# HKUDS/LLMRec

Measured on AMD Instinct MI355X. Metric: bpr_train_edges_per_sec, higher is better.
Workload: dtype f32

## Files before the change

include/llmrec_hip.h:

```cpp
#ifndef LLMREC_HIP_H
#define LLMREC_HIP_H

#include <stdint.h>

#ifdef __cplusplus
extern "C" {
#endif

#define LLMREC_ABI_VERSION 8

enum {
    LLMREC_OK = 0,
    LLMREC_EINVAL = -1,
    LLMREC_EHIP = -2,
    LLMREC_EWORKSPACE = -3,
    LLMREC_EUNSUPPORTED = -4
};

typedef void* llmrec_stream_t;

int llmrec_abi_version(void);
const char* llmrec_status_string(int status);
const char* llmrec_last_error(void);

// ... 27 lines not shown
    int32_t op; float alpha;
    const float* Z; int64_t ldz;
    const float* S; int64_t lds;
    const float* post_scale;
    const uint8_t* x_row_mask; int32_t x_mask_active; uint8_t* y_row_flag; const uint8_t* z_row_flag; const uint8_t* y_row_gate;
    const uint8_t* y_row_needed; int32_t rows_listed_only;
    const int32_t* x_mask_stamp; int32_t mask_from_slice;
} llmrec_spmm_epilogue_t;
#define LLMREC_SORT_UNIQUE_MAX 32768
#define LLMREC_SPMM_COMPACT_PARTS 8
int llmrec_sort_unique_ids_i32(int64_t n, const int64_t* ids, int32_t* list, int32_t* n_out, llmrec_stream_t stream);
int64_t llmrec_spmm_rows_compact_workspace_bytes(int64_t capacity, int32_t d);
int llmrec_spmm_rows_compact_f32(int64_t n_rows, int64_t n_cols, const int32_t* rowptr, const int32_t* colidx, const float* row_scale,
                                 const float* X, int64_t ldx, int32_t d, const int32_t* row_list, const int32_t* n_list_dev, int32_t capacity,
                                 float* out, int64_t ldo, void* workspace, int64_t workspace_bytes, llmrec_stream_t stream);
int llmrec_scatter_set_rows_f32(int32_t capacity, const int32_t* row_list, const int32_t* n_list_dev, int32_t d, const float* src, int64_t lds,
                                float* dst, int64_t ldd, llmrec_stream_t stream);
int llmrec_mark_rows_u8(int64_t n, const int64_t* ids, int32_t value, uint8_t* flags, llmrec_stream_t stream);
int llmrec_mark_neighbours_u8(int64_t n, const int64_t* ids, const int32_t* rowptr, const int32_t* colidx, int32_t value, uint8_t* flags,
                              llmrec_stream_t stream);
int llmrec_batch_reach_rows(int64_t n_users, int64_t n_items, const int64_t* users, const int64_t* pos, const int64_t* neg, int32_t B_cap,
                            const int32_t* n_valid, const int32_t* item_rowptr, const int32_t* item_colidx, uint8_t* flags,
                            int32_t* row_list, int32_t* n_rows, llmrec_stream_t stream);

int llmrec_spmm_plan_count(int64_t n_rows, const int32_t* rowptr, int32_t t_wave, int32_t t_block, int32_t segment,
                           int32_t* scratch4 , int32_t* counts_host, llmrec_stream_t stream);
int llmrec_spmm_plan_fill(int64_t n_rows, const int32_t* rowptr, int32_t t_wave, int32_t t_block, int32_t segment,
                          int32_t* scratch4, int32_t* wave_rows, int32_t* block_rows, int32_t* split_rows,
                          int32_t* split_seg_begin, int32_t* seg_split, llmrec_stream_t stream);

int llmrec_csr_permute_rows(int64_t n_rows, const int32_t* rowptr, const int32_t* colidx, const int32_t* perm, const int32_t* p_rowptr,
                            int32_t* p_colidx, llmrec_stream_t stream);

int llmrec_spmm_f32(int64_t n_rows, int64_t n_cols,
                    const int32_t* rowptr, const int32_t* colidx, const float* val,
                    const float* row_scale, const float* col_scale,
                    const float* X, int64_t ldx, float* Y, int64_t ldy, int32_t d, int32_t slice_width,
                    const llmrec_spmm_plan_t* plan_host, float* partials,
                    const llmrec_spmm_epilogue_t* epilogue_host , llmrec_stream_t stream);

int llmrec_rows_to_bf16(int64_t n_rows, int32_t d, const float* row_scale ,
                        const float* X, int64_t ldx, uint16_t* Xb, int64_t ldxb, llmrec_stream_t stream);
int llmrec_spmm_xbf16_f32(int64_t n_rows, int64_t n_cols, const int32_t* rowptr, const int32_t* colidx, const float* val,
                          const float* row_scale, const float* col_scale,
                          const uint16_t* Xb, int64_t ldxb,
                          float* Y, int64_t ldy,
// ... 437 lines not shown
```

llmrec_amd/csrc/guests.h:

```cpp
#pragma once
#include "common.h"
#include "reach.h"

namespace llmrec {

__device__ __forceinline__ int bpr_batch(const int32_t* n_valid_dev, int B_max) {
    int B = n_valid_dev ? n_valid_dev[0] : B_max;
    return B > B_max ? B_max : (B < 0 ? 0 : B);
}

struct Philox {
    uint32_t key[2];
    __device__ Philox(uint64_t seed) { key[0] = (uint32_t)seed; key[1] = (uint32_t)(seed >> 32); }
    __device__ void operator()(uint32_t c0, uint32_t c1, uint32_t c2, uint32_t c3, uint32_t out[4]) const {
        uint32_t k0 = key[0], k1 = key[1];
#pragma unroll
        for (int r = 0; r < 10; ++r) {
            const uint64_t p0 = (uint64_t)0xD2511F53u * c0, p1 = (uint64_t)0xCD9E8D57u * c2;
            const uint32_t n0 = (uint32_t)(p1 >> 32) ^ c1 ^ k0, n1 = (uint32_t)p1;
            const uint32_t n2 = (uint32_t)(p0 >> 32) ^ c3 ^ k1, n3 = (uint32_t)p0;
            c0 = n0; c1 = n1; c2 = n2; c3 = n3;
            k0 += 0x9E3779B9u; k1 += 0xBB67AE85u;
        }
        out[0] = c0; out[1] = c1; out[2] = c2; out[3] = c3;
// ... 186 lines not shown
        below += kj < me; lower_id += idj < id; same_id += idj == id;
    }
    below = (int)group_sum<16>((float)below); lower_id = (int)group_sum<16>((float)lower_id); same_id = (int)group_sum<16>((float)same_id);
    if (gl == 0) {
        const int base = items ? B_max : 0;
        plan[base + below] = me;
        int32_t* runlen = reinterpret_cast<int32_t*>(plan + 3 * (int64_t)B_max);
        runlen[base + below] = (below == lower_id && id != PLAN_NO_ID) ? same_id : 0;
    }
}

struct PlanReachArgs {
    const int64_t* users;
    const int64_t* pos;
    const int64_t* neg;
    int B_max;
    const int32_t* n_valid_dev;
    uint64_t* plan;
    int plan_blocks;
    int64_t n_users, n_items;
    const int32_t* item_rowptr;
    const int32_t* item_colidx;
    uint8_t* flags;
};

template <int NT>
__device__ __forceinline__ void guest_block(const PlanReachArgs& a, int vb, char* smem) {
    if (vb < a.plan_blocks)
        bpr_plan_block<NT>(vb, reinterpret_cast<uint64_t*>(smem), a.users, a.pos, a.neg, a.B_max, a.n_valid_dev, a.plan);
    else
        batch_reach_mark_block<NT>(vb - a.plan_blocks, a.B_max, a.n_valid_dev, a.users, a.pos, a.neg, a.n_users, a.n_items, a.item_rowptr,
                                   a.item_colidx, a.flags);
}

static inline int guest_prepare(const llmrec_guest_plan_reach_t& g, int nt, const char* who, PlanReachArgs& a, int64_t& blocks, size_t& shmem) {
    blocks = 0; shmem = 0;
    LLMREC_CHECK_ARG(g.B_max >= 0 && g.n_users > 0 && g.n_users < 0x7fffffffll && g.n_items > 0, "%s: bad sizes", who);
    LLMREC_CHECK_ARG(g.item_rowptr && g.item_colidx && g.flags, "%s: null pointer", who);
    if (g.B_max > LLMREC_BPR_MAX_B) { set_error("%s: B_max %d > %d", who, g.B_max, LLMREC_BPR_MAX_B); return LLMREC_EUNSUPPORTED; }
    if (g.B_max == 0) return LLMREC_OK;
    LLMREC_CHECK_ARG(g.users && g.pos && g.neg && g.plan, "%s: null pointer", who);
    const int plan_blocks = (int)plan_blocks_for(g.B_max, nt);
    blocks = plan_blocks + reach_mark_blocks(g.B_max, nt);
    shmem = sizeof(uint64_t) * 2 * (size_t)g.B_max;
    a = PlanReachArgs{g.users, g.pos, g.neg, g.B_max, g.n_valid_dev, g.plan, plan_blocks, g.n_users, g.n_items, g.item_rowptr, g.item_colidx,
                      g.flags};
    return LLMREC_OK;
}

struct LossW { float w[LLMREC_BPR_MAX_PROBLEMS]; };
constexpr int LA_SLOTS = 1024;
constexpr int LA_TREES = 4 * LLMREC_BPR_MAX_PROBLEMS + 1;
__device__ __forceinline__ float wave_tree_sum_1024(const float* __restrict__ src, int n, int lane) {
    float r[16];
#pragma unroll
    for (int j = 0; j < 16; ++j) r[j] = 0.f;
    for (int base = 0; base < n; base += LA_SLOTS) {
        float x[16];
#pragma unroll
        for (int j = 0; j < 16; ++j) { const int b = base + lane + 64 * j; x[j] = b < n ? src[b] : 0.f; }
#pragma unroll
        for (int j = 0; j < 16; ++j) { const int b = base + lane + 64 * j; if (b < n) r[j] += x[j]; }
    }
#pragma unroll
    for (int h = 8; h > 0; h >>= 1) {
#pragma unroll
        for (int j = 0; j < h; ++j) r[j] += r[j + h];
    }
    float x = r[0];
// ... 89 lines not shown
```

llmrec_amd/csrc/reach.h:

```cpp
#pragma once
#include "common.h"

namespace llmrec {

constexpr int REACH_SPLIT = 8;

static inline int64_t reach_mark_blocks(int B_cap, int nt = 256) { return ceil_div(3 * (int64_t)B_cap * REACH_SPLIT, nt / 64); }

template <int NT = 256>
__device__ __forceinline__ void batch_reach_mark_block(int vb, int B_cap, const int32_t* __restrict__ n_valid, const int64_t* __restrict__ users,
                                                       const int64_t* __restrict__ pos, const int64_t* __restrict__ neg, int64_t n_users,
                                                       int64_t n_items, const int32_t* __restrict__ rowptr, const int32_t* __restrict__ colidx,
                                                       uint8_t* __restrict__ flags) {
    const int w = vb * (NT / 64) + (threadIdx.x >> 6), lane = threadIdx.x & 63;
    int nv = n_valid ? *n_valid : B_cap;
    nv = nv < B_cap ? nv : B_cap;
    const int part = w % REACH_SPLIT, job = w / REACH_SPLIT;
    const int b = job / 3, role = job - 3 * b;
    if (b >= nv) return;
    if (role == 0) {
        const int64_t u = users[b];
        if (part == 0 && lane == 0 && u >= 0 && u < n_users) flags[u] = 1;
        return;
    }
    const int64_t it = role == 1 ? pos[b] : neg[b];
    if (it < 0 || it >= n_items) return;
    const int32_t s = rowptr[it], e = rowptr[it + 1];
    for (int32_t k = s + part * 64 + lane; k < e; k += 64 * REACH_SPLIT) flags[colidx[k]] = 1;
}

}
```

llmrec_amd/csrc/rowops.hip:

```cpp
#include "common.h"
#include "adamw.h"
#include "reach.h"
#include <type_traits>

namespace llmrec {

constexpr int RL = 16;
constexpr int ROWS_PER_BLOCK = 256 / RL;

template <int VEC, int NCHUNK>
struct RowReg {
    float x[NCHUNK][VEC];
    __device__ __forceinline__ void load(const float* row, int gl, int d) {
#pragma unroll
        for (int k = 0; k < NCHUNK; ++k) {
            const int c = (k * RL + gl) * VEC;
            if (VEC == 4) {
                float4 v = (c < d) ? *reinterpret_cast<const float4*>(row + c) : make_float4(0.f, 0.f, 0.f, 0.f);
                x[k][0] = v.x; x[k][1 % VEC] = v.y; x[k][2 % VEC] = v.z; x[k][3 % VEC] = v.w;
            } else {
                x[k][0] = (c < d) ? row[c] : 0.f;
            }
        }
    }
    __device__ __forceinline__ void store(float* row, int gl, int d) const {
#pragma unroll
// ... 580 lines not shown
    for (int c = gl; c < d; c += 16) dot = fmaf(y[c], alpha * g[c], dot);
    dot = group_sum<16>(dot);
    const float ps = post_scale ? post_scale[row] : 1.0f;
    float* o = dZ + row * lddz;
    for (int c = gl; c < d; c += 16) o[c] = ps * (y[c] * (alpha * g[c] - dot));
}

constexpr int MARK_SPLIT = 32;
__global__ __launch_bounds__(256) void mark_neighbours_kernel(int64_t n, const int64_t* __restrict__ ids, const int32_t* __restrict__ rowptr,
                                                              const int32_t* __restrict__ colidx, uint8_t value, uint8_t* __restrict__ flags) {
    const int64_t w = (int64_t)blockIdx.x * 4 + (threadIdx.x >> 6);
    const int64_t j = w / MARK_SPLIT;
    const int part = (int)(w - j * MARK_SPLIT);
    if (j >= n) return;
    const int64_t row = ids[j];
    if (row < 0) return;
    const int32_t s = rowptr[row], e = rowptr[row + 1];
    for (int64_t k = (int64_t)s + part * 64 + (threadIdx.x & 63); k < e; k += 64 * MARK_SPLIT) flags[colidx[k]] = value;
}

__global__ __launch_bounds__(256) void batch_reach_mark_kernel(int B_cap, const int32_t* __restrict__ n_valid, const int64_t* __restrict__ users,
                                                               const int64_t* __restrict__ pos, const int64_t* __restrict__ neg, int64_t n_users,
                                                               int64_t n_items, const int32_t* __restrict__ rowptr, const int32_t* __restrict__ colidx,
                                                               uint8_t* __restrict__ flags) {
    batch_reach_mark_block((int)blockIdx.x, B_cap, n_valid, users, pos, neg, n_users, n_items, rowptr, colidx, flags);
}

__global__ __launch_bounds__(1024) void flags_compact_kernel(int64_t n, uint8_t* __restrict__ flags, int32_t* __restrict__ list, int32_t* __restrict__ n_out) {
    __shared__ int32_t wave_total[16];
    const int tid = threadIdx.x, lane = tid & 63, wave = tid >> 6;
    const int64_t per = ((n + 1023) / 1024 + 15) / 16 * 16;
    const int64_t r0 = tid * per, r1 = r0 + per < n ? r0 + per : n;
    int32_t c = 0;
    for (int64_t r = r0; r < r1; r += 16) {
        const uint4 v = *reinterpret_cast<const uint4*>(flags + r);
        const uint32_t wd[4] = {v.x, v.y, v.z, v.w};
#pragma unroll
        for (int q = 0; q < 4; ++q)
#pragma unroll
            for (int bb = 0; bb < 4; ++bb)
                c += (r + 4 * q + bb < r1) && ((wd[q] >> (8 * bb)) & 0xffu);
    }
    int32_t incl = c;
#pragma unroll
    for (int off = 1; off < 64; off <<= 1) {
        const int32_t v = __shfl_up(incl, off, 64);
        if (lane >= off) incl += v;
    }
    if (lane == 63) wave_total[wave] = incl;
    __syncthreads();
    int32_t base = 0, total = 0;
#pragma unroll
// ... 60 lines not shown
            for (int j = 0; j < COMPACT_WPT; ++j) {
                const uint32_t wd[4] = {v[j].x, v[j].y, v[j].z, v[j].w};
                if ((wd[0] | wd[1] | wd[2] | wd[3]) == 0u) continue;
                const int64_t r = 16 * (mine + j);
#pragma unroll
                for (int q = 0; q < 4; ++q)
#pragma unroll
                    for (int bb = 0; bb < 4; ++bb)
                        if ((wd[q] >> (8 * bb)) & 0xffu) list[o++] = (int32_t)(r + 4 * q + bb);
                const int64_t left = n - r;
                if (left >= 16) *reinterpret_cast<uint4*>(flags + r) = uint4{0u, 0u, 0u, 0u};
                else for (int64_t bb = 0; bb < left; ++bb) flags[r + bb] = 0;
            }
        }
        done += total;
    }
    const int32_t pad_end = (done + 15) / 16 * 16 + 16;
    for (int32_t k = done + tid; k < pad_end; k += 256) list[k] = 0;
    if (tid == 0) *n_out = done;
}

template <int VEC, int NCHUNK>
__global__ __launch_bounds__(256) void fuse_fwd_multi_compact_kernel(int d, FuseMulti m, int64_t n_flags, uint8_t* __restrict__ flags,
                                                                     int32_t* __restrict__ list, int32_t* __restrict__ n_out) {
    __shared__ float ss_red[256];
    if (blockIdx.x == 0) { flags_compact_block256(n_flags, flags, list, n_out, reinterpret_cast<int32_t*>(ss_red)); return; }
    fuse_fwd_multi_block<VEC, NCHUNK>((int)blockIdx.x - 1, (int)gridDim.x - 1, d, m, ss_red);
}

constexpr int COLSUM_BLOCKS = 128;
constexpr int COLSUM_MAX_D = 64 * LLMREC_COLSUM_MAX_GROUPS;
__global__ __launch_bounds__(256) void colsum_partial_kernel(int64_t rows, int d, const float* __restrict__ X, int64_t ldx,
                                                             const float* __restrict__ w, float* __restrict__ partial) {
    float acc[COLSUM_MAX_D / 256] = {};
    for (int64_t r = blockIdx.x; r < rows; r += gridDim.x) {
        const float wr = w ? w[r] : 1.f;
        const float* row = X + r * ldx;
#pragma unroll
        for (int k = 0; k < COLSUM_MAX_D / 256; ++k) {
            const int c = k * 256 + threadIdx.x;
            if (c < d) acc[k] = fmaf(wr, row[c], acc[k]);
        }
    }
#pragma unroll
    for (int k = 0; k < COLSUM_MAX_D / 256; ++k) {
        const int c = k * 256 + threadIdx.x;
        if (c < d) partial[(int64_t)blockIdx.x * d + c] = acc[k];
    }
}
struct ColsumGroups { float* out[LLMREC_COLSUM_MAX_GROUPS]; int n_groups; };
// ... 13 lines not shown
    __syncthreads();
    if (c >= gw) return;
    for (int q = 0; q < g.n_groups; ++q) {
        bool first = true;
        for (int e = 0; e < q; ++e) first = first && g.out[e] != g.out[q];
        float* o = g.out[q] + c;
        *o = (first && !accumulate) ? col[gw * q + c] : *o + col[gw * q + c];
    }
}

struct GatherTerms { const float* t[LLMREC_MAX_TERMS]; int64_t ld[LLMREC_MAX_TERMS]; int n; };

__global__ __launch_bounds__(256) void gather_mean_kernel(int64_t n, const int64_t* __restrict__ idx, int d, float scale, GatherTerms g,
                                                          float* __restrict__ out, int64_t ldo) {
    const int gl = threadIdx.x & 15;
    const int64_t b = (int64_t)blockIdx.x * 16 + (threadIdx.x >> 4);
    if (b >= n) return;
    const int64_t row = idx[b];
    for (int c = gl; c < d; c += 16) {
        float s = 0.f;
        for (int t = 0; t < g.n; ++t) s += g.t[t][row * g.ld[t] + c];
        out[b * ldo + c] = scale * s;
    }
}

extern "C" {

int llmrec_softmax_rows_fwd_f32(int64_t rows, int32_t d, const float* Z, int64_t ldz, float* Y, int64_t ldy,
                                llmrec_stream_t stream_) {
    hipStream_t stream = (hipStream_t)stream_;
    LLMREC_CHECK_ARG(rows >= 0 && d > 0, "softmax_fwd: bad sizes");
    if (rows == 0) return LLMREC_OK;
    LLMREC_CHECK_ARG(Z && Y && ldz >= d && ldy >= d, "softmax_fwd: null pointer or ld < d");
    const bool vec4 = d % 4 == 0 && ldz % 4 == 0 && ldy % 4 == 0 && aligned16(Z) && aligned16(Y);
    const int grid = grid_for(rows, ROWS_PER_BLOCK);
    int rc = dispatch_rows(d, vec4,
        [&](auto nc) { softmax_fwd_kernel<4, decltype(nc)::value><<<grid, 256, 0, stream>>>(rows, d, Z, ldz, Y, ldy); return 0; },
        [&](auto nc) { softmax_fwd_kernel<1, decltype(nc)::value><<<grid, 256, 0, stream>>>(rows, d, Z, ldz, Y, ldy); return 0; });
    if (rc) return rc;
    LLMREC_LAUNCH_CHECK();
    return LLMREC_OK;
}

int llmrec_softmax_rows_bwd_scaled_f32(int64_t rows, int32_t d, float alpha, const float* Y, int64_t ldy, const float* dY, int64_t lddy,
                                       float* dZ, int64_t lddz, llmrec_stream_t stream_) {
    hipStream_t stream = (hipStream_t)stream_;
// ... 123 lines not shown
        vec4 = vec4 && q.ldo % 4 == 0 && aligned16(q.out);
        for (int i = 0; i < q.n_mean; ++i) {
            LLMREC_CHECK_ARG(q.mean_terms[i] && q.mean_ld[i] >= d, "fuse_fwd_multi: problem %d: bad mean term %d", k, i);
            a.mean_terms[i] = q.mean_terms[i]; a.mean_ld[i] = q.mean_ld[i];
            vec4 = vec4 && q.mean_ld[i] % 4 == 0 && aligned16(q.mean_terms[i]);
        }
        for (int i = 0; i < q.n_norm; ++i) {
            LLMREC_CHECK_ARG(q.norm_terms[i] && q.norm_ld[i] >= d, "fuse_fwd_multi: problem %d: bad norm term %d", k, i);
            a.norm_terms[i] = q.norm_terms[i]; a.norm_ld[i] = q.norm_ld[i]; a.rates[i] = q.rates[i];
            vec4 = vec4 && q.norm_ld[i] % 4 == 0 && aligned16(q.norm_terms[i]);
        }
        m.rows[k] = q.rows; m.out[k] = q.out; m.ldo[k] = q.ldo;
        blocks[k] = q.rows > 0 ? grid_for(q.rows, ROWS_PER_BLOCK) : 0;
    }
    m.block_begin = blocks[0];
    const int grid = blocks[0] + blocks[1];
    if (n_sumsq_terms > 0) {
        for (int k = 0; k < n_problems; ++k) LLMREC_CHECK_ARG(n_sumsq_terms <= p[k].n_norm, "fuse_fwd_multi: problem %d has fewer than %d norm terms", k, n_sumsq_terms);
        if (grid > partial_capacity) { set_error("fuse_fwd_multi: %d partial sums > capacity %d", grid, partial_capacity); return LLMREC_EWORKSPACE; }
        *n_partial_host = grid;
        m.n_sumsq = n_sumsq_terms; m.sumsq_partial = sumsq_partial;
    }
    if (flags) {
        int rc = dispatch_rows(d, vec4,
            [&](auto nc) { fuse_fwd_multi_compact_kernel<4, decltype(nc)::value><<<grid + 1, 256, 0, stream>>>(d, m, n_flags, flags, row_list, n_rows); return 0; },
            [&](auto) { set_error("fuse_fwd_multi_sumsq_compact: d = %d with rows that are not 16-byte aligned", d); return (int)LLMREC_EUNSUPPORTED; });
        if (rc) return rc;
        LLMREC_LAUNCH_CHECK();
        return LLMREC_OK;
    }
    if (grid == 0) return LLMREC_OK;
    int rc = dispatch_rows(d, vec4,
        [&](auto nc) { fuse_fwd_multi_kernel<4, decltype(nc)::value><<<grid, 256, 0, stream>>>(d, m); return 0; },
        [&](auto nc) { fuse_fwd_multi_kernel<1, decltype(nc)::value><<<grid, 256, 0, stream>>>(d, m); return 0; });
    if (rc) return rc;
    LLMREC_LAUNCH_CHECK();
    return LLMREC_OK;
}

int llmrec_fuse_fwd_multi_sumsq_f32(int32_t n_problems, const llmrec_fuse_fwd_problem_t* p, int32_t d, int32_t n_sumsq_terms,
                                    float* sumsq_partial, int32_t partial_capacity, int32_t* n_partial_host, llmrec_stream_t stream_) {
    return fuse_fwd_multi_launch(n_problems, p, d, n_sumsq_terms, sumsq_partial, partial_capacity, n_partial_host, 0, nullptr, nullptr, nullptr,
                                 (hipStream_t)stream_);
}

int llmrec_fuse_fwd_multi_sumsq_compact_f32(int32_t n_problems, const llmrec_fuse_fwd_problem_t* p, int32_t d, int32_t n_sumsq_terms,
                                            float* sumsq_partial, int32_t partial_capacity, int32_t* n_partial_host,
                                            int64_t n_users, uint8_t* flags, int32_t* row_list, int32_t* n_rows, llmrec_stream_t stream_) {
// ... 231 lines not shown
    LLMREC_CHECK_ARG(row_list && n_list_dev && src && dst && lds_ >= d && ldd >= d, "scatter_set_rows: null pointer or ld < d");
    scatter_set_rows_kernel<<<(unsigned)ceil_div(capacity, 16), 256, 0, (hipStream_t)stream_>>>(capacity, row_list, n_list_dev, d, src, lds_, dst, ldd);
    LLMREC_LAUNCH_CHECK();
    return LLMREC_OK;
}

int llmrec_mark_rows_u8(int64_t n, const int64_t* ids, int32_t value, uint8_t* flags, llmrec_stream_t stream_) {
    LLMREC_CHECK_ARG(n >= 0 && value >= 0 && value <= 255, "mark_rows: bad argument");
    if (n == 0) return LLMREC_OK;
    LLMREC_CHECK_ARG(ids && flags, "mark_rows: null pointer");
    LLMREC_CHECK_ARG(n / 256 < 0x7fffffffll, "mark_rows: too many rows for one launch");
    mark_rows_kernel<<<(unsigned)ceil_div(n, 256), 256, 0, (hipStream_t)stream_>>>(n, ids, (uint8_t)value, flags);
    LLMREC_LAUNCH_CHECK();
    return LLMREC_OK;
}

int llmrec_batch_reach_rows(int64_t n_users, int64_t n_items, const int64_t* users, const int64_t* pos, const int64_t* neg, int32_t B_cap,
                            const int32_t* n_valid, const int32_t* item_rowptr, const int32_t* item_colidx, uint8_t* flags,
                            int32_t* row_list, int32_t* n_rows, llmrec_stream_t stream_) {
    LLMREC_CHECK_ARG(n_users > 0 && n_users < 0x7fffffffll && n_items > 0 && B_cap >= 0, "batch_reach_rows: bad sizes");
    LLMREC_CHECK_ARG(users && pos && neg && item_rowptr && item_colidx && flags && row_list && n_rows, "batch_reach_rows: null pointer");
    LLMREC_CHECK_ARG((uintptr_t)flags % 16 == 0, "batch_reach_rows: flags must be 16-byte aligned (and readable up to n_users rounded up to 16 bytes)");
    hipStream_t stream = (hipStream_t)stream_;
    if (B_cap > 0) {
        batch_reach_mark_kernel<<<(unsigned)reach_mark_blocks(B_cap), 256, 0, stream>>>(B_cap, n_valid, users, pos, neg, n_users, n_items,
                                                                                                item_rowptr, item_colidx, flags);
        LLMREC_LAUNCH_CHECK();
    }
    flags_compact_kernel<<<1, 1024, 0, stream>>>(n_users, flags, row_list, n_rows);
    LLMREC_LAUNCH_CHECK();
    return LLMREC_OK;
}

int llmrec_softmax_rows_bwd_listed_f32(int64_t n, const int64_t* ids, int32_t d, float alpha, const float* Y, int64_t ldy,
                                       const float* dY, int64_t lddy, const float* post_scale, float* dZ, int64_t lddz,
                                       llmrec_stream_t stream_) {
    LLMREC_CHECK_ARG(n >= 0 && d > 0, "softmax_bwd_listed: bad sizes");
    if (n == 0) return LLMREC_OK;
    LLMREC_CHECK_ARG(ids && Y && dY && dZ && ldy >= d && lddy >= d && lddz >= d, "softmax_bwd_listed: null pointer or ld < d");
    softmax_bwd_listed_kernel<<<(unsigned)ceil_div(n, 16), 256, 0, (hipStream_t)stream_>>>(n, ids, d, alpha, Y, ldy, dY, lddy, post_scale, dZ, lddz);
    LLMREC_LAUNCH_CHECK();
    return LLMREC_OK;
}

int llmrec_mark_neighbours_u8(int64_t n, const int64_t* ids, const int32_t* rowptr, const int32_t* colidx, int32_t value, uint8_t* flags,
                              llmrec_stream_t stream_) {
    LLMREC_CHECK_ARG(n >= 0 && value >= 0 && value <= 255, "mark_neighbours: bad argument");
    if (n == 0) return LLMREC_OK;
    LLMREC_CHECK_ARG(ids && rowptr && colidx && flags, "mark_neighbours: null pointer");
    LLMREC_CHECK_ARG(n * MARK_SPLIT / 4 < 0x7fffffffll, "mark_neighbours: too many rows for one launch");
    mark_neighbours_kernel<<<(unsigned)ceil_div(n * MARK_SPLIT, 4), 256, 0, (hipStream_t)stream_>>>(n, ids, rowptr, colidx, (uint8_t)value, flags);
    LLMREC_LAUNCH_CHECK();
    return LLMREC_OK;
// ... 85 lines not shown
```

llmrec_amd/fused.py:

```python
from __future__ import annotations

import contextlib
import ctypes
import gc
from collections import namedtuple
from itertools import zip_longest
from typing import Callable, Optional

import torch

from . import _lib, ops, step_options
from .engine import Hyper

_p, _ld, _c = ops._p, ops._ld, ctypes


def _call(name, *a):
    _lib.call(name, *a, ops._stream())


def _raw(args):
    return [_p(a) if a is None or isinstance(a, torch.Tensor) else a for a in args]


@contextlib.contextmanager
def _capture_without_gc(graph, multi_branch: bool):
    from . import require_graph_replay
# ... 130 lines not shown
        if self.restore:
            if decoder is None or user_targets is None or item_targets is None or feat_loss_type not in ops.RESTORE_LOSS_TYPES:
                raise RuntimeError("FusedStep: the restoration term needs the decoder, both target sets and feat_loss_type sce or mse")
            if d != 64 or S > 2 + _lib.CONST["LLMREC_MASK_MAX_TENSORS"]:
                raise RuntimeError("FusedStep: the restoration launches are compiled for d = 64 and at most %d attribute streams"
                                   % _lib.CONST["LLMREC_MASK_MAX_TENSORS"])
            as_target = lambda x: torch.as_tensor(x).detach().to(device=dev, dtype=torch.float32).contiguous()
            self.decoder, self.feat_loss_type, self.alpha_l = decoder, feat_loss_type, float(alpha_l)
            self.user_targets, self.item_targets = as_target(user_targets), [as_target(item_targets[k]) for k in self.keys]
            self.re_rows_u, self.re_rows_i = f(self.m_users), f(len(self.keys) * self.m_items)
            self.re_vals = z(1 + len(self.keys))
        if not self.preprop:
            self.P_cat, self.dP_cat = f(I, S * d), f(I, S * d)
        else:
            item_feats = [model.image_feats, model.text_feats] + [model.item_feats[k] for k in self.keys]
            self.AX = [self._propagate_constant(self.ui.fwd, x) for x in item_feats]
            self.a_rowsum = ops.spmm_raw(self.ui.fwd, torch.ones(I, 4, dtype=torch.float32, device=dev))[:, 0].contiguous()
            self.ws_colsum = torch.empty(_lib.query("llmrec_weighted_colsum_workspace_bytes", S * d), dtype=torch.uint8, device=dev)
        if self.wgrad_rows:
            self.act_flags = torch.zeros(U + 16, dtype=torch.uint8, device=dev)[:U]
            self.act_rows = torch.zeros(U + 32, dtype=torch.int32, device=dev)
            self.act_n = torch.zeros(1, dtype=torch.int32, device=dev)
            self.act_expected = None
        if self.fold:
            self.ss_cap = 2 * 2048
            self.ss_partial = torch.zeros(self.ss_cap, dtype=torch.float32, device=dev)
            self.ss_n = 0
        self._refuse_guests = False
        self._block_slots = 2 * torch.cuda.get_device_properties(dev).multi_processor_count
        self._emb_params = [model.user_id_embedding.weight, model.item_id_embedding.weight]
        self._lin_params = [p for p in optimizer.params if p.grad is not None and all(p is not e for e in self._emb_params)]

    @staticmethod
    def _propagate_constant(a: ops.Csr, X: torch.Tensor) -> torch.Tensor:
        X = X.detach()
        out = torch.empty(a.n_rows, X.shape[1], dtype=torch.float32, device=X.device)
        step = 64 if X.shape[1] % 64 == 0 else X.shape[1]
        for c0 in range(0, X.shape[1], step):
            ops.spmm_raw(a, X[:, c0:c0 + step], out=out[:, c0:c0 + step])
        return out

    def _fork(self, *streams):
        if self.multi_stream:
            cur = torch.cuda.current_stream()
            for st in streams:
                st.wait_stream(cur)
# ... 90 lines not shown
    def _linear(self, X, lin, out):
        _call("llmrec_linear_fwd_f32", X.shape[0], self.d, X.shape[1], _p(X), _ld(X), _p(lin.weight), _ld(lin.weight), _p(lin.bias),
              _p(out), _ld(out))

    def projection_jobs(self):
        m = self.m
        if self.preprop:
            lins = [m.image_trans, m.text_trans] + [m.item_trans] * len(self.keys)
            jobs = [(self.AX[s_], lins[s_], self._side(self.U_cat, s_), self.a_rowsum) for s_ in range(self.S)]
        else:
            jobs = [(m.item_feats[key], m.item_trans, self._side(self.P_cat, 2 + k), None) for k, key in enumerate(self.keys)]
            jobs += [(m.text_feats, m.text_trans, self._side(self.P_cat, 1), None), (m.image_feats, m.image_trans, self._side(self.P_cat, 0), None)]
        jobs.append((m.user_feats, m.user_trans, self.P_usr, None))
        jobs.sort(key=lambda j: -j[0].shape[1])
        return jobs

    def wgrad_targets(self, dY_cat, dP_usr):
        m = self.m
        if self.preprop:
            feats, roww = self.AX, self.a_rowsum
        else:
            feats, roww = [m.image_feats, m.text_feats] + [m.item_feats[key] for key in self.keys], None
        rows = (self.act_rows, self.act_n, self.act_expected) if self.wgrad_rows else None
        item_pairs = [(self._side(dY_cat, 2 + k), feats[2 + k], roww, rows) for k in range(len(self.keys))]
        return [(item_pairs, m.item_trans.weight.grad, m.item_trans.bias.grad, False),
                ([(dP_usr, m.user_feats)], m.user_trans.weight.grad, m.user_trans.bias.grad, False),
                ([(self._side(dY_cat, 1), feats[1], roww)], m.text_trans.weight.grad, m.text_trans.bias.grad, False),
                ([(self._side(dY_cat, 0), feats[0], roww)], m.image_trans.weight.grad, m.image_trans.bias.grad, False)]

    def _project_all(self):
        jobs = self.projection_jobs()
        if self.d > 64 or len(jobs) > _lib.CONST["LLMREC_LINEAR_MAX_PROBLEMS"]:
            if self.preprop:
                raise RuntimeError("FusedStep: the pre-propagated projection needs the grouped launch (d <= 64); set LLMREC_PREPROPAGATE=0")
            for X, lin, out, _ in jobs:
                self._linear(X, lin, out)
            return
        arr = self._projection_problems(jobs)
        _call("llmrec_linear_fwd_grouped_bf16x3" if self.gemm == "bf16x3" else "llmrec_linear_fwd_grouped_f32", len(jobs), arr, self.d)

    @staticmethod
    def _projection_problems(jobs):
        return ops.linear_problems([(X, lin.weight, lin.bias, out, bscale) for X, lin, out, bscale in jobs])

    def _project_all_hosting(self, job) -> bool:
        a, X, Y, kw = job
        jobs = self.projection_jobs()
        if not (self.host_chain and not self._refuse_guests and not self.multi_stream and self.gemm == "bf16x3" and self.d == 64
                and len(jobs) <= _lib.CONST["LLMREC_LINEAR_MAX_PROBLEMS"] and a.nnz < ops.SPMM_LATENCY_NNZ
# ... 441 lines not shown
        if main_first:
            self._spmm_jobs(side)
            self._fork_from(ev_fuse, self.s1)
        else:
            self._fork(self.s1)
        if loss_s3:
            self._fork_from(ev_rows, self.s3)
            with self._on(self.s3):
                side_work()
            side_work = None
        with self._on(self.s1):
            self._spmm_jobs(prof)
            if self.gemm != "bf16x3" and not self.drop_rate > 0:
                self._wgrad(self.dP_usr, self.m.user_feats, self.m.user_trans, False, ws=self.ws_wgrad_b)
        self._fork_from(ev_rows, self.s2)
        with self._on(self.s2):
            self._chain_head(side_work)
            self._spmm_jobs(self._chain_bwd_jobs())
            self._chain_tail(probs, batch, ev_fuse)
        if not main_first:
            self._spmm_jobs(side)
        self._check_mask_promise(masked, done=True)

    def _weight_gradients(self, ev_reach=None, deferred=None):
        m, S, d = self.m, self.S, self.d
        hosted = deferred[0][0] if deferred is not None else None
        dY_cat = self.dU_cat if self.preprop else self.dP_cat
        targets = self.wgrad_targets(dY_cat, self.dP_usr)
        item_pairs, text_pairs, image_pairs = targets[0][0], targets[2][0], targets[3][0]
        done, updated = False, []
        if self.gemm == "bf16x3":
            self._join(self.s1)
            if self._wgrad_multi_workspace(targets) is not False:
                self._stamp(3)
                if ev_reach is not None:
                    torch.cuda.current_stream().wait_event(ev_reach)
                lins = (m.item_trans, m.user_trans, m.text_trans, m.image_trans)
                if self.inline_adamw:
                    update = (self.opt, [(l.weight, l.bias) for l in lins])
                    accepted = False
                    if hosted is not None:
                        probs, keep = self._spmm_problems([hosted])
                        accepted = ops.linear_wgrad_multi(targets, self.ws_wgrad_multi, update=update, block_budget=self.wgrad_blocks,
                                                          host_spmm=(probs[0], self._block_slots // 2))
                        del keep
                        if accepted:
                            self.spmm_edge_units += hosted[0].nnz * (hosted[1].shape[1] / 64.0)
                        else:
                            self._spmm_jobs([hosted])
                        hosted = None
                    if not accepted:
                        ops.linear_wgrad_multi(targets, self.ws_wgrad_multi, update=update, block_budget=self.wgrad_blocks)
                    updated = [p_ for l in lins for p_ in (l.weight, l.bias)]
                else:
                    ops.linear_wgrad_multi(targets, self.ws_wgrad_multi, block_budget=self.wgrad_blocks)
# ... 61 lines not shown
        self.spmm_edge_units = 0.0
        calls0 = _lib.n_calls
        try:
            self._stamp(0)
            if self.multi_stream or step.ride:
                self._train_forward(sampler, batch_lists, step)
            else:
                if sampler is not None:
                    sampler()
                batch_lists()
                self._train_forward(step=step)
            self.loss_backward(users, pos, neg, n_valid, step)
            if not self.inline_adamw:
                self.opt.step(advanced=True)
            self._stamp(5)
            self.entry_point_calls_per_step = _lib.n_calls - calls0 - (2 if self.stamps is not None else 0) * 3
            if self.wgrad_rows and self.act_expected is None and not torch.cuda.is_current_stream_capturing():
                self._size_wgrad_for_rows()
        except Exception:
            if not torch.cuda.is_current_stream_capturing():
                with contextlib.suppress(Exception):
                    if step.reach_pending is not None:
                        self.act_flags.zero_()
                    self.reset_scatter_targets()
            raise
        return self.scal[1], self.scal[2], self.scal[3]

    def _size_wgrad_for_rows(self, expected: Optional[int] = None):
        if expected is not None:
            self.act_expected = expected
        else:
            n = int(self.act_n.item())
            self.act_expected = max(64, min(self.U, int(n * 1.10) + 32))
        need = ops.linear_wgrad_multi_workspace(self.wgrad_targets(self.dU_cat if self.preprop else self.dP_cat, self.dP_usr), self.wgrad_blocks)
        self.ws_wgrad_multi = torch.empty(max(need, 0), dtype=torch.uint8, device=self.dP_usr.device) if need >= 0 else False

    def check_wgrad_geometry(self, factor: float = 1.5) -> bool:
        if not self.wgrad_rows or self.act_expected is None or torch.cuda.is_current_stream_capturing():
            return False
        want = max(64, min(self.U, int(int(self.act_n.item()) * 1.10) + 32))
        if self.act_expected / factor <= want <= self.act_expected * factor:
            return False
        self._size_wgrad_for_rows()
        if self.graph_exec is not None and self._capture_args is not None:
            self.capture(warm=False, **self._capture_args)
        return True

    def flush(self):
        """Nothing is deferred in the single-graph step (DataParallelStep defers its AdamW)."""

    def state_tensors(self):
        from .engine import model_state_tensors
        out = model_state_tensors(self.m, self.opt)
        out += [("step/row_stamp", self.row_stamp), ("step/flag_u", self.flag_u), ("step/flag_i", self.flag_i), ("step/epoch_sums", self.epoch_sums)]
        if self.drop_rate > 0:
            out += [("step/drop_step", self.drop_step), ("step/drop_ticket", self.drop_ticket)]
        if self.mask_rate > 0:
            out += [("step/mask_step", self.mask_step), ("step/mask_ticket", self.mask_ticket)]
            out += [("step/user_sums/%d" % k, t) for k, t in enumerate(self.user_sums)]
            out += [("step/item_sums/%d" % k, t) for k, t in enumerate(self.item_sums)]
        if self.restore:
            out += [("decoder/" + name, p.data) for name, p in self.decoder.named_parameters()]
        return out

    def host_state(self):
        return {"act_expected": self.act_expected if self.wgrad_rows else None}

    replayed_mask_rounds = None

    def prepare_load(self, saved):
        if not self.mask_rate > 0:
            return
        import time
        want = saved("step/mask_step")
        if want is None:
            raise RuntimeError("FusedStep.prepare_load: the checkpoint holds no masking state")
        if int(self.mask_step.view(torch.int64).item()) != 0:
            raise RuntimeError("FusedStep.prepare_load: this step has already masked its features (mask_step != 0); a masking checkpoint "
                               "loads into a fresh step only")
        rounds = int(want.view(torch.int64).item())
        t0 = time.perf_counter()
        for _ in range(rounds):
            self._mask_round()
        torch.cuda.current_stream().synchronize()
        self.replayed_mask_rounds = (rounds, time.perf_counter() - t0)
        mine = dict(self.state_tensors())
        bad = [name for name in mine if name.startswith(("step/mask_step", "step/user_sums/", "step/item_sums/"))
               and not torch.equal(mine[name].view(torch.int64), saved(name).view(torch.int64))]
        if bad:
            raise RuntimeError("FusedStep.prepare_load: %d replayed masking rounds do not reproduce the saved %s (other features, "
                               "another seed or mask_rate?)" % (rounds, bad))

    def finish_load(self, host):
        expected = (host or {}).get("act_expected")
        if self.wgrad_rows and expected is not None and expected != self.act_expected:
            self._size_wgrad_for_rows(int(expected))
            if self.graph_exec is not None and self._capture_args is not None:
                self.capture(warm=False, **self._capture_args)

    @torch.no_grad()
    def load_state(self, saved, host=None):
        self.prepare_load(saved)
        for name, t in self.state_tensors():
            src = saved(name)
            if src is None or src.shape != t.shape or src.dtype != t.dtype:
                raise RuntimeError("FusedStep.load_state: %s is missing from the saved state or has another shape / dtype" % name)
            t.copy_(src)
        self.finish_load(host)

    def eval_topk(self, query_users: torch.Tensor, train: Optional[ops.Csr], K: int, use_graph: bool = False, held=None, Ks=None,
                  auc: bool = False):
        if auc and (not use_graph or held is None):
            raise RuntimeError("FusedStep.eval_topk: auc=True needs use_graph=True and the held-out rows")
        if not use_graph:
            self.forward()
            return ops.score_topk(self.E_u, self.E_i, query_users, train, K)
        Ks = tuple(int(k) for k in Ks) if held is not None else None
        key = (query_users.data_ptr(), query_users.numel(), K, id(train), None if held is None else (held[0].data_ptr(), Ks), bool(auc))
        ev = self._eval_graphs.get(key)
# ... 153 lines not shown
```

Baseline: 2.237 million.

## Restrict user-side weight gradient to two-hop reachable user rows

Adds a second reachability set covering batch users, users of pos/neg items, and users two hops away through each batch user's items. This row list feeds the user_trans weight-gradient GEMM so it only touches rows where dP_usr can be nonzero, instead of all users. It costs extra marking work per batch (a fourth role per sample that walks user→item→user neighbourhoods), an extra compaction block, and a host-side lookup table keyed by flag pointer.

Measured after the change: 1.829 million. 0.817x the previous value.

```diff
diff --git a/include/llmrec_hip.h b/include/llmrec_hip.h
--- a/include/llmrec_hip.h
+++ b/include/llmrec_hip.h
@@ -73,6 +73,9 @@
 int llmrec_batch_reach_rows(int64_t n_users, int64_t n_items, const int64_t* users, const int64_t* pos, const int64_t* neg, int32_t B_cap,
                             const int32_t* n_valid, const int32_t* item_rowptr, const int32_t* item_colidx, uint8_t* flags,
                             int32_t* row_list, int32_t* n_rows, llmrec_stream_t stream);
+int llmrec_reach_two_hop_attach(uint8_t* flags, int64_t n_users, const int32_t* user_rowptr, const int32_t* user_colidx, uint8_t* flags2,
+                                int32_t* row_list2, int32_t* n_rows2);
+int llmrec_reach_two_hop_detach(const uint8_t* flags);
 
 int llmrec_spmm_plan_count(int64_t n_rows, const int32_t* rowptr, int32_t t_wave, int32_t t_block, int32_t segment,
                            int32_t* scratch4 , int32_t* counts_host, llmrec_stream_t stream);
diff --git a/llmrec_amd/csrc/guests.h b/llmrec_amd/csrc/guests.h
--- a/llmrec_amd/csrc/guests.h
+++ b/llmrec_amd/csrc/guests.h
@@ -232,12 +232,16 @@
     const int32_t* item_rowptr;
     const int32_t* item_colidx;
     uint8_t* flags;
+    ReachTwoHop two;
 };
 
 template <int NT>
 __device__ __forceinline__ void guest_block(const PlanReachArgs& a, int vb, char* smem) {
     if (vb < a.plan_blocks)
         bpr_plan_block<NT>(vb, reinterpret_cast<uint64_t*>(smem), a.users, a.pos, a.neg, a.B_max, a.n_valid_dev, a.plan);
+    else if (a.two.flags2)
+        batch_reach_mark_two_hop_block<NT>(vb - a.plan_blocks, a.B_max, a.n_valid_dev, a.users, a.pos, a.neg, a.n_users, a.n_items, a.item_rowptr,
+                                           a.item_colidx, a.flags, a.two);
     else
         batch_reach_mark_block<NT>(vb - a.plan_blocks, a.B_max, a.n_valid_dev, a.users, a.pos, a.neg, a.n_users, a.n_items, a.item_rowptr,
                                    a.item_colidx, a.flags);
@@ -251,10 +255,13 @@
     if (g.B_max == 0) return LLMREC_OK;
     LLMREC_CHECK_ARG(g.users && g.pos && g.neg && g.plan, "%s: null pointer", who);
     const int plan_blocks = (int)plan_blocks_for(g.B_max, nt);
-    blocks = plan_blocks + reach_mark_blocks(g.B_max, nt);
+    ReachTwoHop two;
+    const bool two_hop = reach_two_hop_of(g.flags, two);
+    LLMREC_CHECK_ARG(!two_hop || two.n_users == g.n_users, "%s: the attached two-hop set is for another n_users", who);
+    blocks = plan_blocks + reach_mark_blocks(g.B_max, nt, two_hop);
     shmem = sizeof(uint64_t) * 2 * (size_t)g.B_max;
     a = PlanReachArgs{g.users, g.pos, g.neg, g.B_max, g.n_valid_dev, g.plan, plan_blocks, g.n_users, g.n_items, g.item_rowptr, g.item_colidx,
-                      g.flags};
+                      g.flags, two};
     return LLMREC_OK;
 }
 
diff --git a/llmrec_amd/csrc/reach.h b/llmrec_amd/csrc/reach.h
--- a/llmrec_amd/csrc/reach.h
+++ b/llmrec_amd/csrc/reach.h
@@ -5,7 +5,19 @@
 
 constexpr int REACH_SPLIT = 8;
 
-static inline int64_t reach_mark_blocks(int B_cap, int nt = 256) { return ceil_div(3 * (int64_t)B_cap * REACH_SPLIT, nt / 64); }
+struct ReachTwoHop {
+    const int32_t* user_rowptr;
+    const int32_t* user_colidx;
+    uint8_t* flags2;
+    int32_t* row_list2;
+    int32_t* n_rows2;
+    int64_t n_users;
+};
+bool reach_two_hop_of(const uint8_t* flags, ReachTwoHop& t);
+
+static inline int64_t reach_mark_blocks(int B_cap, int nt = 256, bool two_hop = false) {
+    return ceil_div((two_hop ? 4 : 3) * (int64_t)B_cap * REACH_SPLIT, nt / 64);
+}
 
 template <int NT = 256>
 __device__ __forceinline__ void batch_reach_mark_block(int vb, int B_cap, const int32_t* __restrict__ n_valid, const int64_t* __restrict__ users,
@@ -29,4 +41,43 @@
     for (int32_t k = s + part * 64 + lane; k < e; k += 64 * REACH_SPLIT) flags[colidx[k]] = 1;
 }
 
+template <int NT = 256>
+__device__ __forceinline__ void batch_reach_mark_two_hop_block(int vb, int B_cap, const int32_t* __restrict__ n_valid, const int64_t* __restrict__ users,
+                                                               const int64_t* __restrict__ pos, const int64_t* __restrict__ neg, int64_t n_users,
+                                                               int64_t n_items, const int32_t* __restrict__ rowptr,
+                                                               const int32_t* __restrict__ colidx, uint8_t* flags, const ReachTwoHop& two) {
+    const int w = vb * (NT / 64) + (threadIdx.x >> 6), lane = threadIdx.x & 63;
+    int nv = n_valid ? *n_valid : B_cap;
+    nv = nv < B_cap ? nv : B_cap;
+    const int part = w % REACH_SPLIT, job = w / REACH_SPLIT;
+    const int b = job >> 2, role = job & 3;
+    uint8_t* flags2 = two.flags2;
+    if (b >= nv) return;
+    if (role == 0) {
+        const int64_t u = users[b];
+        if (part == 0 && lane == 0 && u >= 0 && u < n_users) { flags[u] = 1; flags2[u] = 1; }
+        return;
+    }
+    if (role == 3) {
+        const int64_t u = users[b];
+        if (u < 0 || u >= n_users) return;
+        const int32_t us = two.user_rowptr[u], ue = two.user_rowptr[u + 1];
+        for (int32_t j = us + part; j < ue; j += REACH_SPLIT) {
+            const int32_t it = two.user_colidx[j];
+            if (it < 0 || it >= n_items) continue;
+            const int32_t s = rowptr[it], e = rowptr[it + 1];
+            for (int32_t k = s + lane; k < e; k += 64) flags2[colidx[k]] = 1;
+        }
+        return;
+    }
+    const int64_t it = role == 1 ? pos[b] : neg[b];
+    if (it < 0 || it >= n_items) return;
+    const int32_t s = rowptr[it], e = rowptr[it + 1];
+    for (int32_t k = s + part * 64 + lane; k < e; k += 64 * REACH_SPLIT) {
+        const int32_t u = colidx[k];
+        flags[u] = 1;
+        flags2[u] = 1;
+    }
 }
+
+}
diff --git a/llmrec_amd/csrc/rowops.hip b/llmrec_amd/csrc/rowops.hip
--- a/llmrec_amd/csrc/rowops.hip
+++ b/llmrec_amd/csrc/rowops.hip
@@ -1,7 +1,10 @@
 #include "common.h"
 #include "adamw.h"
 #include "reach.h"
+#include <mutex>
 #include <type_traits>
+#include <utility>
+#include <vector>
 
 namespace llmrec {
 
@@ -628,12 +631,15 @@
 __global__ __launch_bounds__(256) void batch_reach_mark_kernel(int B_cap, const int32_t* __restrict__ n_valid, const int64_t* __restrict__ users,
                                                                const int64_t* __restrict__ pos, const int64_t* __restrict__ neg, int64_t n_users,
                                                                int64_t n_items, const int32_t* __restrict__ rowptr, const int32_t* __restrict__ colidx,
-                                                               uint8_t* __restrict__ flags) {
-    batch_reach_mark_block((int)blockIdx.x, B_cap, n_valid, users, pos, neg, n_users, n_items, rowptr, colidx, flags);
-}
-
-__global__ __launch_bounds__(1024) void flags_compact_kernel(int64_t n, uint8_t* __restrict__ flags, int32_t* __restrict__ list, int32_t* __restrict__ n_out) {
+                                                               uint8_t* __restrict__ flags, ReachTwoHop two) {
+    if (two.flags2) batch_reach_mark_two_hop_block((int)blockIdx.x, B_cap, n_valid, users, pos, neg, n_users, n_items, rowptr, colidx, flags, two);
+    else batch_reach_mark_block((int)blockIdx.x, B_cap, n_valid, users, pos, neg, n_users, n_items, rowptr, colidx, flags);
+}
+
+__global__ __launch_bounds__(1024) void flags_compact_kernel(int64_t n, uint8_t* __restrict__ flags, int32_t* __restrict__ list, int32_t* __restrict__ n_out,
+                                                             uint8_t* __restrict__ flags2, int32_t* __restrict__ list2, int32_t* __restrict__ n_out2) {
     __shared__ int32_t wave_total[16];
+    if (blockIdx.x == 1) { flags = flags2; list = list2; n_out = n_out2; }
     const int tid = threadIdx.x, lane = tid & 63, wave = tid >> 6;
     const int64_t per = ((n + 1023) / 1024 + 15) / 16 * 16;
     const int64_t r0 = tid * per, r1 = r0 + per < n ? r0 + per : n;
@@ -740,10 +746,14 @@
 
 template <int VEC, int NCHUNK>
 __global__ __launch_bounds__(256) void fuse_fwd_multi_compact_kernel(int d, FuseMulti m, int64_t n_flags, uint8_t* __restrict__ flags,
-                                                                     int32_t* __restrict__ list, int32_t* __restrict__ n_out) {
+                                                                     int32_t* __restrict__ list, int32_t* __restrict__ n_out,
+                                                                     uint8_t* __restrict__ flags2, int32_t* __restrict__ list2,
+                                                                     int32_t* __restrict__ n_out2) {
     __shared__ float ss_red[256];
+    const int lead = flags2 ? 2 : 1;
     if (blockIdx.x == 0) { flags_compact_block256(n_flags, flags, list, n_out, reinterpret_cast<int32_t*>(ss_red)); return; }
-    fuse_fwd_multi_block<VEC, NCHUNK>((int)blockIdx.x - 1, (int)gridDim.x - 1, d, m, ss_red);
+    if (blockIdx.x == 1 && flags2) { flags_compact_block256(n_flags, flags2, list2, n_out2, reinterpret_cast<int32_t*>(ss_red)); return; }
+    fuse_fwd_multi_block<VEC, NCHUNK>((int)blockIdx.x - lead, (int)gridDim.x - lead, d, m, ss_red);
 }
 
 constexpr int COLSUM_BLOCKS = 128;
@@ -803,6 +813,17 @@
         for (int t = 0; t < g.n; ++t) s += g.t[t][row * g.ld[t] + c];
         out[b * ldo + c] = scale * s;
     }
+}
+
+static std::mutex two_hop_mutex;
+static std::vector<std::pair<const uint8_t*, ReachTwoHop>> two_hop_table;
+
+bool llmrec::reach_two_hop_of(const uint8_t* flags, ReachTwoHop& t) {
+    t = ReachTwoHop{};
+    std::lock_guard<std::mutex> lock(two_hop_mutex);
+    for (const auto& e : two_hop_table)
+        if (e.first == flags) { t = e.second; return true; }
+    return false;
 }
 
 extern "C" {
@@ -972,8 +993,12 @@
         m.n_sumsq = n_sumsq_terms; m.sumsq_partial = sumsq_partial;
     }
     if (flags) {
+        ReachTwoHop two;
+        const bool two_hop = reach_two_hop_of(flags, two);
+        LLMREC_CHECK_ARG(!two_hop || two.n_users == n_flags, "fuse_fwd_multi_sumsq_compact: the attached two-hop set is for another n_users");
         int rc = dispatch_rows(d, vec4,
-            [&](auto nc) { fuse_fwd_multi_compact_kernel<4, decltype(nc)::value><<<grid + 1, 256, 0, stream>>>(d, m, n_flags, flags, row_list, n_rows); return 0; },
+            [&](auto nc) { fuse_fwd_multi_compact_kernel<4, decltype(nc)::value><<<grid + (two_hop ? 2 : 1), 256, 0, stream>>>(
+                               d, m, n_flags, flags, row_list, n_rows, two.flags2, two.row_list2, two.n_rows2); return 0; },
             [&](auto) { set_error("fuse_fwd_multi_sumsq_compact: d = %d with rows that are not 16-byte aligned", d); return (int)LLMREC_EUNSUPPORTED; });
         if (rc) return rc;
         LLMREC_LAUNCH_CHECK();
@@ -1251,13 +1276,36 @@
     LLMREC_CHECK_ARG(users && pos && neg && item_rowptr && item_colidx && flags && row_list && n_rows, "batch_reach_rows: null pointer");
     LLMREC_CHECK_ARG((uintptr_t)flags % 16 == 0, "batch_reach_rows: flags must be 16-byte aligned (and readable up to n_users rounded up to 16 bytes)");
     hipStream_t stream = (hipStream_t)stream_;
+    ReachTwoHop two;
+    const bool two_hop = reach_two_hop_of(flags, two);
+    LLMREC_CHECK_ARG(!two_hop || two.n_users == n_users, "batch_reach_rows: the attached two-hop set is for another n_users");
     if (B_cap > 0) {
-        batch_reach_mark_kernel<<<(unsigned)reach_mark_blocks(B_cap), 256, 0, stream>>>(B_cap, n_valid, users, pos, neg, n_users, n_items,
-                                                                                                item_rowptr, item_colidx, flags);
+        batch_reach_mark_kernel<<<(unsigned)reach_mark_blocks(B_cap, 256, two_hop), 256, 0, stream>>>(B_cap, n_valid, users, pos, neg, n_users,
+                                                                                                      n_items, item_rowptr, item_colidx, flags, two);
         LLMREC_LAUNCH_CHECK();
     }
-    flags_compact_kernel<<<1, 1024, 0, stream>>>(n_users, flags, row_list, n_rows);
-    LLMREC_LAUNCH_CHECK();
+    flags_compact_kernel<<<two_hop ? 2 : 1, 1024, 0, stream>>>(n_users, flags, row_list, n_rows, two.flags2, two.row_list2, two.n_rows2);
+    LLMREC_LAUNCH_CHECK();
+    return LLMREC_OK;
+}
+
+int llmrec_reach_two_hop_attach(uint8_t* flags, int64_t n_users, const int32_t* user_rowptr, const int32_t* user_colidx, uint8_t* flags2,
+                                int32_t* row_list2, int32_t* n_rows2) {
+    LLMREC_CHECK_ARG(n_users > 0 && n_users < 0x7fffffffll, "reach_two_hop_attach: bad sizes");
+    LLMREC_CHECK_ARG(flags && user_rowptr && user_colidx && flags2 && row_list2 && n_rows2 && flags2 != flags, "reach_two_hop_attach: null pointer");
+    LLMREC_CHECK_ARG((uintptr_t)flags2 % 16 == 0, "reach_two_hop_attach: flags2 must be 16-byte aligned (and readable up to n_users rounded up to 16 bytes)");
+    const ReachTwoHop t = {user_rowptr, user_colidx, flags2, row_list2, n_rows2, n_users};
+    std::lock_guard<std::mutex> lock(two_hop_mutex);
+    for (auto& e : two_hop_table)
+        if (e.first == flags) { e.second = t; return LLMREC_OK; }
+    two_hop_table.emplace_back(flags, t);
+    return LLMREC_OK;
+}
+
+int llmrec_reach_two_hop_detach(const uint8_t* flags) {
+    std::lock_guard<std::mutex> lock(two_hop_mutex);
+    for (size_t i = 0; i < two_hop_table.size(); ++i)
+        if (two_hop_table[i].first == flags) { two_hop_table.erase(two_hop_table.begin() + (long)i); break; }
     return LLMREC_OK;
 }
 
diff --git a/llmrec_amd/fused.py b/llmrec_amd/fused.py
--- a/llmrec_amd/fused.py
+++ b/llmrec_amd/fused.py
@@ -3,6 +3,7 @@
 import contextlib
 import ctypes
 import gc
+import weakref
 from collections import namedtuple
 from itertools import zip_longest
 from typing import Callable, Optional
@@ -179,6 +180,13 @@
             self.act_rows = torch.zeros(U + 32, dtype=torch.int32, device=dev)
             self.act_n = torch.zeros(1, dtype=torch.int32, device=dev)
             self.act_expected = None
+            self.act2_flags = torch.zeros(U + 16, dtype=torch.uint8, device=dev)[:U]
+            self.act2_rows = torch.zeros(U + 32, dtype=torch.int32, device=dev)
+            self.act2_n = torch.zeros(1, dtype=torch.int32, device=dev)
+            self.act2_expected = None
+            _lib.call("llmrec_reach_two_hop_attach", _p(self.act_flags), U, _p(self.ui.fwd.rowptr), _p(self.ui.fwd.colidx), _p(self.act2_flags),
+                  _p(self.act2_rows), _p(self.act2_n))
+            weakref.finalize(self, _lib.call, "llmrec_reach_two_hop_detach", self.act_flags.data_ptr())
         if self.fold:
             self.ss_cap = 2 * 2048
             self.ss_partial = torch.zeros(self.ss_cap, dtype=torch.float32, device=dev)
@@ -315,9 +323,10 @@
         else:
             feats, roww = [m.image_feats, m.text_feats] + [m.item_feats[key] for key in self.keys], None
         rows = (self.act_rows, self.act_n, self.act_expected) if self.wgrad_rows else None
+        rows2 = (self.act2_rows, self.act2_n, self.act2_expected) if self.wgrad_rows else None
         item_pairs = [(self._side(dY_cat, 2 + k), feats[2 + k], roww, rows) for k in range(len(self.keys))]
         return [(item_pairs, m.item_trans.weight.grad, m.item_trans.bias.grad, False),
-                ([(dP_usr, m.user_feats)], m.user_trans.weight.grad, m.user_trans.bias.grad, False),
+                ([(dP_usr, m.user_feats, None, rows2)], m.user_trans.weight.grad, m.user_trans.bias.grad, False),
                 ([(self._side(dY_cat, 1), feats[1], roww)], m.text_trans.weight.grad, m.text_trans.bias.grad, False),
                 ([(self._side(dY_cat, 0), feats[0], roww)], m.image_trans.weight.grad, m.image_trans.bias.grad, False)]
 
@@ -805,6 +814,15 @@
             self._spmm_jobs(side)
         self._check_mask_promise(masked, done=True)
 
+    def _check_two_hop_promise(self):
+        if not (self.wgrad_rows and self.check_zero) or torch.cuda.is_current_stream_capturing():
+            return
+        torch.cuda.synchronize()
+        idle = torch.ones(self.U, dtype=torch.bool, device=self.dP_usr.device)
+        idle[self.act2_rows[:int(self.act2_n.item())].long()] = False
+        if idle.any() and float(self.dP_usr[idle].abs().max()) != 0.0:
+            raise RuntimeError("FusedStep: dP_usr is not all-zero outside the two-hop row list")
+
     def _weight_gradients(self, ev_reach=None, deferred=None):
         m, S, d = self.m, self.S, self.d
         hosted = deferred[0][0] if deferred is not None else None
@@ -814,6 +832,7 @@
         done, updated = False, []
         if self.gemm == "bf16x3":
             self._join(self.s1)
+            self._check_two_hop_promise()
             if self._wgrad_multi_workspace(targets) is not False:
                 self._stamp(3)
                 if ev_reach is not None:
@@ -921,24 +940,28 @@
                 with contextlib.suppress(Exception):
                     if step.reach_pending is not None:
                         self.act_flags.zero_()
+                        self.act2_flags.zero_()
                     self.reset_scatter_targets()
             raise
         return self.scal[1], self.scal[2], self.scal[3]
 
     def _size_wgrad_for_rows(self, expected: Optional[int] = None):
         if expected is not None:
-            self.act_expected = expected
-        else:
-            n = int(self.act_n.item())
-            self.act_expected = max(64, min(self.U, int(n * 1.10) + 32))
+            self.act_expected, self.act2_expected = expected
+        else:
+            n, n2 = (int(v) for v in torch.cat([self.act_n, self.act2_n]).tolist())
+            self.act_expected, self.act2_expected = self._rows_to_lay_out(n), self._rows_to_lay_out(n2)
         need = ops.linear_wgrad_multi_workspace(self.wgrad_targets(self.dU_cat if self.preprop else self.dP_cat, self.dP_usr), self.wgrad_blocks)
         self.ws_wgrad_multi = torch.empty(max(need, 0), dtype=torch.uint8, device=self.dP_usr.device) if need >= 0 else False
+
+    def _rows_to_lay_out(self, n: int) -> int:
+        return max(64, min(self.U, int(n * 1.10) + 32))
 
     def check_wgrad_geometry(self, factor: float = 1.5) -> bool:
         if not self.wgrad_rows or self.act_expected is None or torch.cuda.is_current_stream_capturing():
             return False
-        want = max(64, min(self.U, int(int(self.act_n.item()) * 1.10) + 32))
-        if self.act_expected / factor <= want <= self.act_expected * factor:
+        n, n2 = (int(v) for v in torch.cat([self.act_n, self.act2_n]).tolist())
+        if all(have / factor <= self._rows_to_lay_out(v) <= have * factor for v, have in ((n, self.act_expected), (n2, self.act2_expected))):
             return False
         self._size_wgrad_for_rows()
         if self.graph_exec is not None and self._capture_args is not None:
@@ -963,7 +986,8 @@
         return out
 
     def host_state(self):
-        return {"act_expected": self.act_expected if self.wgrad_rows else None}
+        on = self.wgrad_rows
+        return {"act_expected": self.act_expected if on else None, "act2_expected": self.act2_expected if on else None}
 
     replayed_mask_rounds = None
 
@@ -991,9 +1015,11 @@
                                "another seed or mask_rate?)" % (rounds, bad))
 
     def finish_load(self, host):
-        expected = (host or {}).get("act_expected")
-        if self.wgrad_rows and expected is not None and expected != self.act_expected:
-            self._size_wgrad_for_rows(int(expected))
+        expected, expected2 = (host or {}).get("act_expected"), (host or {}).get("act2_expected")
+        if self.wgrad_rows and expected is not None and expected2 is None:
+            expected2 = self.act2_expected or self.U
+        if self.wgrad_rows and expected is not None and (expected, expected2) != (self.act_expected, self.act2_expected):
+            self._size_wgrad_for_rows((int(expected), int(expected2)))
             if self.graph_exec is not None and self._capture_args is not None:
                 self.capture(warm=False, **self._capture_args)
 
```
